# LogicTronixInc/Event-Camera-Clustering-and-Optical-Flow-Estimation

Measured on AMD Instinct MI355X. Metric: Mevents/s (downsample+cluster+corner), higher is better.
Workload: dtype u16xy/i64t (int), fp32 k-means; 1 GPU; e2e hash-downsample(8192-event windows) -> k-means k=16 (10 iters) on reps -> SAE+FAST arc corners (16384-event slices) -> 15x15 NMS; 346x260 sensor; 20004864 events/GPU/step (BASELINE configs C2-C4); events_per_gpu=20004864, events_total=20004864, preset=c4, reps_per_gpu=7697279, width=346, height=260, k=16, kmeans_iters=10, parallelism=time-window shards x1, launch=eager launches, streams=two streams sharing all CUs

## Files before the change

### event-camera-clustering-and-optical-flow-estimation_amd/csrc/corners.hip

```cpp
#include "arc_select.hpp"
#include "corner_decode.hpp"
#include "ecc_internal.hpp"

#include <cstdio>
#include <cstdlib>
#include <map>
#include <mutex>

namespace {

constexpr int kThreads = 256;
constexpr int kBuildUnroll = 8;
constexpr size_t kFlagDynLdsMax = 160 * 1024 - 256;
constexpr int kArcThreads = 512;
constexpr int kGroup = 32;
constexpr int kTile = 14;
constexpr int kTilePix = kTile * kTile;
constexpr int kHalo = 4;
constexpr int kWin = kTile + 2 * kHalo;
constexpr int kWinPix = kWin * kWin;
constexpr int kMaxTiles = 8191;
constexpr int kMaxSlice = 1 << 19;

struct CornerGeom {
// ... 13 lines not shown
    tile = (int)((uint32_t)item - q * (uint32_t)g.n_tiles);
}

struct Sorted {
    uint32_t *key;
    uint32_t *t32;
    int32_t *toff;
};

__constant__ int8_t c3dy[16] = {0, 1, 2, 3, 3, 3, 2, 1, 0, -1, -2, -3, -3, -3, -2, -1};
__constant__ int8_t c3dx[16] = {3, 3, 2, 1, 0, -1, -2, -3, -3, -3, -2, -1, 0, 1, 2, 3};
__constant__ int8_t c4dy[20] = {0, 1, 2, 3, 4, 4, 4, 3, 2, 1, 0, -1, -2, -3, -4, -4, -4, -3, -2, -1};
__constant__ int8_t c4dx[20] = {4, 4, 3, 2, 1, 0, -1, -2, -3, -4, -4, -4, -3, -2, -1, 0, 1, 2, 3, 4};

__device__ __forceinline__ bool is_border(int x, int y, const CornerGeom &g) {
    return x < g.margin || x >= g.W - g.margin || y < g.margin || y >= g.H - g.margin;
}

__device__ __forceinline__ int tile_of(uint32_t v, const CornerGeom &g) {
    const int x = ecc::xy_x(v), y = ecc::xy_y(v);
    const int tl = (int)__umul24((uint32_t)(y / kTile), (uint32_t)g.tiles_x) + x / kTile;
    return (x >= g.W || y >= g.H) ? g.n_tiles : tl;
}

__device__ __forceinline__ uint32_t tile_key(uint32_t v, uint32_t e_local) {
    return (e_local << 8) | (uint32_t)((ecc::xy_y(v) % kTile) * kTile + ecc::xy_x(v) % kTile);
}

__device__ __forceinline__ void tile_origin_xy(const CornerGeom &g, int tile, int &tx, int &ty) {
    ty = (int)magic_quot((uint32_t)tile, g.tx_mul, g.tx_sh);
    tx = tile - ty * g.tiles_x;
// ... 393 lines not shown
    uint32_t r0 = 0u, r1 = 0u, r2 = 0u, r3 = x4;
    uint32_t v = 0u;
    int k = 0;
    for (uint32_t mm = m; mm; mm &= mm - 1u, ++k) {
        v = tab[__ffs(mm) - 1][lp];
        if (k == 0) r0 = v;
        else if (k == 1) r1 = v;
        else if (k == 2) r2 = v;
        else if (cnt == kRecVals) r3 = v;
        else xo[k] = v;
    }
    pv[q] = make_uint4(r0, r1, r2, r3);
    glast[q] = gr.narrow ? gr.Lt + (int64_t)v : t[gr.first + v - 1u];
}

constexpr int kPrefixPix = 64;
constexpr int kPrefixPer = 16;
constexpr int kPrefixRound = kPrefixPer * (kThreads / 64);

__global__ void __launch_bounds__(kThreads)
sae_prefix_kernel(CornerGeom g, int64_t n_groups, const uint32_t *__restrict__ gmask, int64_t *__restrict__ gB,
                  int64_t *__restrict__ sae, int32_t *__restrict__ err_status,
                  int32_t *__restrict__ err_pending, int32_t tag,
                  uint32_t *__restrict__ zero0, int32_t *__restrict__ zero1) {
    if (blockIdx.x == 0 && threadIdx.x == 0) {
        *err_status = *err_pending == tag ? 1 : 0;
        *err_pending = 0;
        if (zero0) *zero0 = 0u;
        if (zero1) *zero1 = 0;
    }
    __shared__ int64_t s_last[kThreads / 64][kPrefixPix];
    __shared__ uint8_t s_has[kThreads / 64][kPrefixPix];
    const int lane = threadIdx.x & 63, wave = threadIdx.x >> 6;
    const int64_t HW = (int64_t)g.H * g.W;
    const int64_t q = (int64_t)blockIdx.x * kPrefixPix + lane;
    const bool in = q < HW;
    int64_t carry = in ? sae[q] : 0;
    for (int64_t r0 = 0; r0 < n_groups; r0 += kPrefixRound) {
        const int64_t g0 = r0 + (int64_t)wave * kPrefixPer;
        uint32_t m[kPrefixPer];
        int64_t lt[kPrefixPer];
#pragma unroll
        for (int u = 0; u < kPrefixPer; ++u) m[u] = (in && g0 + u < n_groups) ? gmask[(g0 + u) * HW + q] : 0u;
#pragma unroll
        for (int u = 0; u < kPrefixPer; ++u) lt[u] = m[u] ? gB[(g0 + u) * HW + q] : 0;
        bool has = false;
        int64_t last = 0;
#pragma unroll
        for (int u = 0; u < kPrefixPer; ++u) {
            if (m[u]) { has = true; last = lt[u]; }
        }
        s_last[wave][lane] = last;
        s_has[wave][lane] = has ? 1 : 0;
        __syncthreads();
        int64_t run = carry;
        for (int w = 0; w < wave; ++w)
            if (s_has[w][lane]) run = s_last[w][lane];
#pragma unroll
        for (int u = 0; u < kPrefixPer; ++u) {
            if (!in || g0 + u >= n_groups) break;
            gB[(g0 + u) * HW + q] = run;
            if (m[u]) run = lt[u];
        }
#pragma unroll
        for (int w = 0; w < kThreads / 64; ++w)
            if (s_has[w][lane]) carry = s_last[w][lane];
        __syncthreads();
    }
    if (in && wave == 0) sae[q] = carry;
}

__global__ void __launch_bounds__(kThreads)
sae_local_last_kernel(CornerGeom g, int64_t n_groups, const uint32_t *__restrict__ gmask,
                      const int64_t *__restrict__ glast, int64_t *__restrict__ out) {
    const int64_t HW = (int64_t)g.H * g.W;
    for (int64_t q = (int64_t)blockIdx.x * kThreads + threadIdx.x; q < HW; q += (int64_t)gridDim.x * kThreads) {
        int64_t run = 0;
        for (int64_t gi = n_groups - 1; gi >= 0; --gi)
            if (gmask[gi * HW + q]) { run = glast[gi * HW + q]; break; }
        out[q] = run;
    }
}


constexpr int kPairWords = kGroup * kTilePix / 32;
constexpr int kSegWords = (kTilePix + 31) / 32;

__device__ __forceinline__ void store_res_slice_major(const uint32_t *bits, int64_t grp, int tile, const CornerGeom &g,
                                                      uint32_t *__restrict__ res, int tid) {
    if (tid >= kGroup * kSegWords) return;
    const int j = tid / kSegWords, w = tid % kSegWords;
    const int b0 = j * kTilePix + 32 * w, w0 = b0 >> 5, sh = b0 & 31;
    uint32_t v = bits[w0] >> sh;
    if (sh && w0 + 1 < kPairWords) v |= bits[w0 + 1] << (32 - sh);
    if (w == kSegWords - 1) v &= (1u << (kTilePix - 32 * (kSegWords - 1))) - 1u;
    res[(grp * kGroup + j) * g.seg_stride + tile * kSegWords + w] = v;
}
constexpr int kWaves = kArcThreads / 64;
constexpr int kQ4Cap = 1024;

struct MaskB {
    uint32_t mask;
    uint32_t bc;
};

struct ArcLds {
    uint32_t T[kGroup][kWinPix];
    MaskB mb[kWinPix];
    uint32_t res[kPairWords];
    uint16_t tasks[kGroup * kTilePix];
    uint16_t q4[kQ4Cap];
    int64_t wave_min[16];
    int32_t exact_only;
    int32_t mixed;
    int32_t q4n;
    int32_t n_exact;
    int32_t wave_own[16];
    int32_t wave_tasks[16];
};

__device__ __forceinline__ uint32_t clamp_rel(int64_t v, int64_t L, int64_t vz, int32_t *exact_flag,
                                              int32_t *mixed_flag) {
    if (v <= L) {
        if (v != vz) *mixed_flag = 1;
        return 0u;
    }
    const int64_t d = v - L;
    if (d > (int64_t)kVMax) { *exact_flag = 1; return kVMax; }
    return (uint32_t)d;
}

__device__ __forceinline__ int64_t readlane_i64(int64_t v, int l) {
    return (int64_t)((uint64_t)__builtin_amdgcn_readlane((uint32_t)((uint64_t)v >> 32), l) << 32 |
                     (uint64_t)__builtin_amdgcn_readlane((uint32_t)v, l));
}
__device__ __forceinline__ void clamp_wave_flags(int64_t bq, int64_t Lt, int64_t &c0, int &cf) {
    const bool clp = bq <= Lt;
    const uint64_t cball = __ballot(clp);
    c0 = 0;
    cf = 0;
    if (cball) {
        c0 = readlane_i64(bq, __ffsll((unsigned long long)cball) - 1);
        cf = 2 | (__ballot(clp && bq != c0) != 0ull ? 1 : 0);
    }
}
template <int W>
__device__ __forceinline__ bool clamp_mixed(const int64_t *wc0, const int32_t *wcf, int lane) {
    const int wf = lane < W ? wcf[lane] : 0;
    const int64_t wv = lane < W ? wc0[lane] : 0;
    const uint64_t has = __ballot(wf & 2);
    bool mixed = __ballot(wf & 1) != 0ull;
    if (has) {
        const int64_t v0 = readlane_i64(wv, __ffsll((unsigned long long)has) - 1);
        mixed = mixed || __ballot((wf & 2) && wv != v0) != 0ull;
    }
    return mixed;
}
__device__ __forceinline__ uint32_t clamp_value(int64_t bq, int64_t Lt, bool narrow, int32_t *exact_flag) {
    if (!narrow || bq == INT64_MAX || bq <= Lt) return 0u;
    const int64_t d = bq - Lt;
    if (d > (int64_t)kVMax) {
        *exact_flag = 1;
        return kVMax;
    }
    return (uint32_t)d;
}

__device__ __forceinline__ uint32_t below_mask(int j) { return (2u << j) - 1u; }

__device__ __forceinline__ uint32_t win_value(const ArcLds &L, int wp, uint32_t below) {
    const MaskB m = L.mb[wp];
    const uint32_t mk = m.mask & below;
    return mk ? L.T[31 - __clz(mk)][wp] : m.bc;
}

struct ExactCtx {
    const int64_t *Bg;
    const int64_t *t;
    int64_t grp_first, Lt;
    int W;
    bool narrow;
};

__device__ __forceinline__ int64_t double_key(int64_t v) {
    const int64_t b = __builtin_bit_cast(int64_t, (double)v);
    return b ^ ((b >> 63) & INT64_MAX);
}

template <int N>
__device__ __forceinline__ void exact_values(const ArcLds *L, int wp0, int64_t q0, uint32_t below,
                                             const int8_t *dy, const int8_t *dx, const ExactCtx &c, int64_t (&v)[N]) {
#pragma unroll
    for (int k = 0; k < N; ++k) {
        if (k > 0 && k % 4 == 0) __builtin_amdgcn_sched_barrier(0);
        const int wp = wp0 + dy[k] * kWin + dx[k];
        const uint32_t mk = L->mb[wp].mask & below;
        const uint32_t tv = mk ? L->T[31 - __clz(mk)][wp] : 0u;
        v[k] = double_key(!mk        ? c.Bg[q0 + (int64_t)dy[k] * c.W + dx[k]]
                          : c.narrow ? c.Lt + (int64_t)tv
                                     : c.t[c.grp_first + tv - 1u]);
    }
}


__device__ __noinline__ bool exact_pair_test(const ArcLds *L, int wp0, int64_t q0, uint32_t below, bool c3_passed,
                                             const int64_t *Bg, const int64_t *t, int64_t grp_first, int64_t Lt, int W,
                                             bool narrow) {
    const ExactCtx c{Bg, t, grp_first, Lt, W, narrow};
    if (!c3_passed) {
        int64_t v3[16];
        exact_values<16>(L, wp0, q0, below, c3dy, c3dx, c, v3);
        if (!arc_streak<16, 3, 6>(v3)) return false;
    }
    int64_t v4[20];
    exact_values<20>(L, wp0, q0, below, c4dy, c4dx, c, v4);
    return arc_streak<20, 4, 8>(v4);
}


__device__ __forceinline__ uint32_t eligible_slices(const CornerGeom &g, int64_t grp) {
    const int gs = (int)grp * kGroup;
    if (g.first_detect <= gs) return 0xffffffffu;
    const int j0 = g.first_detect - gs;
// ... 27 lines not shown
#define DENSE_MARK(k)                                                                \
    do {                                                                             \
        if (tid == 0) {                                                              \
            const unsigned long long now_ = wall_clock64();                          \
            atomicAdd(&g_dense_prof[k], now_ - dense_t_);                            \
            dense_t_ = now_;                                                         \
        }                                                                            \
    } while (0)
#else
#define DENSE_MARK(k) do { } while (0)
#endif

template <int NT>
__device__ __forceinline__ void arc_dense_item(ArcLds &L, int64_t item, const int64_t *__restrict__ t, const CornerGeom &g,
                                               const uint32_t *__restrict__ ovf, const uint4 *__restrict__ pv,
                                               const int64_t *__restrict__ gB, const uint32_t *__restrict__ gmask,
                                               uint32_t *__restrict__ res, const GroupRec *__restrict__ grec) {
    int64_t grp;
    int tile;
    item_decode(g, item, grp, tile);
    if ((int)grp < (g.first_detect >> 5)) return;
    const int tid = threadIdx.x, lane = tid & 63, wave = tid >> 6;
#if ECC_ARC_PROFILE
    const unsigned long long dense_t0_ = wall_clock64();
    unsigned long long dense_t_ = dense_t0_;
#endif
    const int64_t HW = (int64_t)g.H * g.W;
    int tx, ty;
    tile_origin_xy(g, tile, tx, ty);
    const int x0 = tx * kTile, y0 = ty * kTile;
    const GroupRef gr = group_ref_of(grec[grp]);
    const int64_t grp_first = gr.first, Lt = gr.Lt;
    const bool narrow = gr.narrow;
    const int64_t *Bg = gB + grp * HW;

    static_assert(NT >= kWinPix, "one lane per window pixel");
    const int wp = tid;
    const bool win_lane = wp < kWinPix;
    const int ox = wp % kWin - kHalo, oy = wp / kWin - kHalo;
    const int wx = x0 + ox, wy = y0 + oy;
    const bool in = win_lane && wx >= 0 && wy >= 0 && wx < g.W && wy < g.H;
    const int64_t q = grp * HW + (int64_t)wy * g.W + wx;
    int64_t bq = INT64_MAX;
    uint32_t mk = 0u;
    uint4 rec = make_uint4(0u, 0u, 0u, 0u);
    if (in) {
        bq = gB[q];
        mk = gmask[q];
        rec = pv[q];
    }
    for (int w = tid; w < kPairWords; w += NT) L.res[w] = 0u;
    if (tid == 0) {
        L.exact_only = narrow ? 0 : 1;
        L.mixed = 0;
        L.q4n = 0;
        L.n_exact = 0;
    }
    const bool own = win_lane && ox >= 0 && oy >= 0 && ox < kTile && oy < kTile;
    const uint64_t own_pairs = __ballot(own && mk != 0u);
    if (lane == 0) L.wave_own[wave] = own_pairs != 0ull;
    const uint32_t tm0 = (own && !is_border(wx, wy, g)) ? (mk & eligible_slices(g, grp)) : 0u;
    const int tcnt = __popc(tm0);
    const int tincl = ecc::wave_incl_scan(tcnt);
    if (lane == 63) L.wave_tasks[wave] = tincl;
    __syncthreads();
    if (win_lane) {
        L.mb[wp].mask = mk;
        const int p = __popc(mk);
        uint32_t mm = mk;
        for (int k = 0; mm && k < kRecVals - 1; ++k, mm &= mm - 1u)
            L.T[__ffs(mm) - 1][wp] = k == 0 ? rec.x : (k == 1 ? rec.y : rec.z);
        if (mm && p == kRecVals) {
            L.T[__ffs(mm) - 1][wp] = rec.w;
        } else if (mm) {
            overflow_lines(ovf, rec, 0, p, [&](int, uint32_t v) {
                L.T[__ffs(mm) - 1][wp] = v;
                mm &= mm - 1u;
            });
        }
    }
    int toff = tincl - tcnt, n_tasks = 0;
#pragma unroll
    for (int w = 0; w < NT / 64; ++w) {
        const int c = L.wave_tasks[w];
        toff += w < wave ? c : 0;
        n_tasks += c;
    }
    for (uint32_t tm = tm0; tm; tm &= tm - 1u) L.tasks[toff++] = (uint16_t)((__ffs(tm) - 1) << 9 | wp);
    const int64_t bmin = ecc::wave_min_i64(bq);
    if (lane == 0) L.wave_min[wave] = bmin;
    __syncthreads();
    DENSE_MARK(0);
    {
        int any = 0;
#pragma unroll
        for (int w = 0; w < NT / 64; ++w) any |= L.wave_own[w];
        if (!any) return;
    }
    DENSE_MARK(1);

    if (win_lane) {
        int64_t vz = INT64_MAX;
#pragma unroll
        for (int w = 0; w < NT / 64; ++w) vz = L.wave_min[w] < vz ? L.wave_min[w] : vz;
        L.mb[wp].bc = (!narrow || bq == INT64_MAX) ? 0u : clamp_rel(bq, Lt, vz, &L.exact_only, &L.mixed);
    }
    __syncthreads();
    DENSE_MARK(2);

    const bool fast = !L.exact_only;
    const bool ties_exact = !L.mixed;
    constexpr uint16_t kOpen3 = 0x4000, kOpen4 = 0x8000;
    if (fast) {
        for (int ti = tid; ti < n_tasks; ti += NT) {
            const int pi = L.tasks[ti];
            const int wp0 = pi & 511;
            const uint32_t below = below_mask(pi >> 9);
            uint32_t k3[16];
#pragma unroll
            for (int k = 0; k < 16; ++k) k3[k] = (win_value(L, wp0 + c3dy[k] * kWin + c3dx[k], below) << 5) | k;
            const int r3 = arc_keys<16, 5, 3, 6>(k3, ties_exact);
            if (r3 > 0) {
                const int qi = atomicAdd(&L.q4n, 1);
                if (qi < kQ4Cap) L.q4[qi] = (uint16_t)ti;
                else { L.tasks[ti] = (uint16_t)(pi | kOpen4); L.n_exact = 1; }
// ... 4 lines not shown
        }
    }
    __syncthreads();
    DENSE_MARK(3);
    const int n4 = min(L.q4n, kQ4Cap);
    for (int qi = tid; qi < n4; qi += NT) {
        const int ti = L.q4[qi];
        const int pi = L.tasks[ti];
        const int j = pi >> 9, wp0 = pi & 511;
        const uint32_t below = below_mask(j);
        uint32_t k4[20];
#pragma unroll
        for (int k = 0; k < 20; ++k) k4[k] = (win_value(L, wp0 + c4dy[k] * kWin + c4dx[k], below) << 5) | k;
        const int r4 = arc_keys<20, 5, 4, 8>(k4, ties_exact);
        if (r4 > 0) {
            const int rb = j * kTilePix + (wp0 / kWin - kHalo) * kTile + (wp0 % kWin - kHalo);
            atomicOr(&L.res[rb >> 5], 1u << (rb & 31));
        } else if (r4 < 0) {
            L.tasks[ti] = (uint16_t)(pi | kOpen4);
            L.n_exact = 1;
        }
    }
    __syncthreads();
    DENSE_MARK(4);
    if (!fast || L.n_exact) {
        for (int ti = tid; ti < n_tasks; ti += NT) {
            const int e = L.tasks[ti], pi = e & 0x3fff;
            if (fast && !(e & (kOpen3 | kOpen4))) continue;
            const int j = pi >> 9, wp0 = pi & 511;
            const int ly = wp0 / kWin - kHalo, lx = wp0 % kWin - kHalo;
            const int64_t q0 = (int64_t)(y0 + ly) * g.W + (x0 + lx);
            const uint32_t below = below_mask(j);
            if (exact_pair_test(&L, wp0, q0, below, (e & kOpen4) != 0, Bg, t, grp_first, Lt, g.W, narrow)) {
                const int rb = j * kTilePix + ly * kTile + lx;
                atomicOr(&L.res[rb >> 5], 1u << (rb & 31));
            }
        }
        __syncthreads();
    }
#if ECC_ARC_PROFILE
    if (tid == 0) {
        atomicMax(&g_dense_prof[5], wall_clock64() - dense_t0_);
        atomicAdd(&g_dense_prof[6], (unsigned long long)n_tasks);
        atomicAdd(&g_dense_prof[7], 1ull);
    }
#endif
    store_res_slice_major(L.res, grp, tile, g, res, tid);
}

// ... 3 lines not shown
constexpr int kValCap = ECC_ARC_VALCAP;

struct PixInfo {
    uint32_t mask;
    uint32_t off;
};

struct SparseLds {
    uint32_t vals[kValCap + kWinPix];
    PixInfo pix[kWinPix];
    uint32_t res[kPairWords];
    uint16_t tasks[kValCap];
    uint16_t q4[kQ4Cap];
    int64_t wave_c0[kWaves];
    int32_t wave_cf[kWaves];
    int32_t wave_tot[kWaves];
    int32_t exact_only, mixed, q4n, redo;
};

static_assert(sizeof(PixInfo) == 8, "one 8-B LDS read per pixel");
__device__ __forceinline__ uint32_t sparse_value(const SparseLds &L, int wp, uint32_t below) {
    const uint2 p = reinterpret_cast<const uint2 *>(L.pix)[wp];
    return L.vals[p.y + __popc(p.x & below)];
}

#ifndef ECC_ARC_SKIP_OVF
#define ECC_ARC_SKIP_OVF 0
#endif
#ifndef ECC_ARC_WAVES
#define ECC_ARC_WAVES 8
#endif

// ... 1 lines not shown
constexpr int kProfItems = 1 << 15;
__device__ unsigned long long g_arc_items[kProfItems][8];
#define ARC_MARK(k)                                                                  \
    do {                                                                             \
        if (tid == 0) {                                                              \
            const unsigned long long now_ = wall_clock64();                          \
            arc_ph_[k] = now_ - arc_t_;                                              \
            arc_t_ = now_;                                                           \
        }                                                                            \
    } while (0)
#else
#define ARC_MARK(k) do { } while (0)
#endif

struct ArcPre {
    int64_t bq;
    uint32_t mk;
    uint4 rec;
};

__device__ __forceinline__ void arc_prefetch(ArcPre &p, int64_t item, const CornerGeom &g, const uint4 *__restrict__ pv,
                                             const int64_t *__restrict__ gB, const uint32_t *__restrict__ gmask) {
    const int tid = threadIdx.x;
    p.bq = INT64_MAX;
    p.mk = 0u;
    p.rec = make_uint4(0u, 0u, 0u, 0u);
    const int64_t HW = (int64_t)g.H * g.W;
    int64_t grp;
    int tile, tx, ty;
    item_decode(g, item, grp, tile);
    tile_origin_xy(g, tile, tx, ty);
    const int wx = tx * kTile - kHalo + tid % kWin, wy = ty * kTile - kHalo + tid / kWin;
    if (tid < kWinPix && wx >= 0 && wy >= 0 && wx < g.W && wy < g.H) {
        const int64_t q = grp * HW + (int64_t)wy * g.W + wx;
        p.bq = gB[q];
        p.mk = gmask[q];
        p.rec = pv[q];
    }
}

__device__ __forceinline__ void arc_item(SparseLds &L, int64_t item, const ArcPre &pre,
                                         const GroupRec *__restrict__ grec, const CornerGeom &g,
                                         const uint32_t *__restrict__ ovf, uint32_t *__restrict__ res,
                                         int64_t *__restrict__ over, uint32_t *__restrict__ n_over) {
    int64_t grp;
    int tile;
    item_decode(g, item, grp, tile);
    if ((int)grp < (g.first_detect >> 5)) return;
    static_assert(kGroup == 32, "first_detect >> 5");
    const int tid = threadIdx.x, lane = tid & 63, wave = tid >> 6;
    const int wave_s = __builtin_amdgcn_readfirstlane(wave);
#if ECC_ARC_PROFILE
    unsigned long long arc_t_ = wall_clock64(), arc_ph_[8] = {0, 0, 0, 0, 0, 0, 0, 0};
#endif
    int tx, ty;
    tile_origin_xy(g, tile, tx, ty);
    const int x0 = tx * kTile, y0 = ty * kTile;
    const GroupRec rec = grec[grp];
    const int64_t Lt = rec.Lt;
    const bool narrow = (rec.bits & kRecNarrow) != 0u;
    const int wp = tid;
    const bool win_lane = wp < kWinPix;
    const int64_t bq = pre.bq;
    const uint32_t mk_w = pre.mk;
    const int ox = wp % kWin - kHalo, oy = wp / kWin - kHalo;
    const bool own = win_lane && ox >= 0 && oy >= 0 && ox < kTile && oy < kTile;
    for (int w = tid; w < kPairWords; w += kArcThreads) L.res[w] = 0u;
    if (tid == 0) {
        L.exact_only = narrow ? 0 : 1;
        L.q4n = 0;
        L.redo = 0;
    }
    const uint32_t tm = (own && !is_border(x0 + ox, y0 + oy, g)) ? (mk_w & eligible_slices(g, grp)) : 0u;
    const int cnt = win_lane ? __popc(mk_w) + 1 : 0;
    const int tcnt = __popc(tm);
    constexpr int kTaskShift = 14, kOwnShift = 27;
    constexpr int kCntMask = (1 << kTaskShift) - 1, kTaskMask = (1 << (kOwnShift - kTaskShift)) - 1;
    const int both = ecc::wave_incl_scan(tcnt << kTaskShift | cnt);
    const int incl = both & kCntMask, tincl = both >> kTaskShift;
    const uint64_t own_pairs = __ballot(own && mk_w != 0u);
    int64_t c0;
    int cf;
    clamp_wave_flags(bq, Lt, c0, cf);
    const int p = cnt - 1;
#ifndef ECC_ARC_XPF
#define ECC_ARC_XPF 1
#endif
    constexpr int kXpf = ECC_ARC_XPF > 0 ? ECC_ARC_XPF : 1;
    uint4 xs[kXpf];
#pragma unroll
    for (int u = 0; u < kXpf; ++u) xs[u] = make_uint4(0u, 0u, 0u, 0u);
    if (ECC_ARC_XPF && __ballot(p > kRecVals)) {
        const bool o = p > kRecVals;
        const uint4 *x4 = reinterpret_cast<const uint4 *>(ovf) + (o ? pre.rec.w : 0u);
        const int nl = o ? (p - (kRecVals - 1) + 3) >> 2 : 1;
#pragma unroll
        for (int u = 0; u < kXpf; ++u) xs[u] = x4[min(u, nl - 1)];
    }
    if (lane == 63) L.wave_tot[wave] = both | (own_pairs != 0ull ? 1 << kOwnShift : 0);
    if (lane == 0) {
        L.wave_c0[wave] = c0;
        L.wave_cf[wave] = cf;
    }
    __syncthreads();
    ARC_MARK(0);
    int sum = 0, before = 0;
#pragma unroll
    for (int w = 0; w < kWaves; ++w) {
        const int wb = L.wave_tot[w];
        sum += wb;
        before += w < wave_s ? wb : 0;
    }
    const int total = sum & kCntMask, any_own = sum >> kOwnShift;
    int n_tasks = (sum >> kTaskShift) & kTaskMask;
    const int off = incl - cnt + (before & kCntMask);
    int toff = tincl - tcnt + ((before >> kTaskShift) & kTaskMask);
    if (wave == 0) {
        const bool mixed = clamp_mixed<kWaves>(L.wave_c0, L.wave_cf, lane);
        if (lane == 0) L.mixed = mixed;
    }
    if (!any_own || total > kValCap + kWinPix) {
        if (any_own && tid == 0) over[atomicAdd(n_over, 1u)] = item;
        return;
    }
    if (win_lane) {
        const uint32_t bcv = clamp_value(bq, Lt, narrow, &L.exact_only);
        reinterpret_cast<uint2 *>(L.pix)[wp] = make_uint2(mk_w, (uint32_t)off);
        uint32_t *dst = L.vals + off;
        dst[0] = bcv;
        if (p > 0) dst[1] = pre.rec.x;
        if (p > 1) dst[2] = pre.rec.y;
        if (p > 2) dst[3] = pre.rec.z;
        if (p == kRecVals) {
            dst[4] = pre.rec.w;
        } else if (!ECC_ARC_XPF && p > kRecVals) {
            overflow_lines(ovf, pre.rec, 0, p, [&](int k, uint32_t v) { dst[1 + k] = v; });
        } else if (p > kRecVals) {
#pragma unroll
            for (int u = 0; u < kXpf; ++u) {
                const int k = (kRecVals - 1) + 4 * u;
                if (k < p) dst[1 + k] = xs[u].x;
                if (k + 1 < p) dst[2 + k] = xs[u].y;
                if (k + 2 < p) dst[3 + k] = xs[u].z;
                if (k + 3 < p) dst[4 + k] = xs[u].w;
            }
            if (!ECC_ARC_SKIP_OVF && p > kRecVals + 4 * ECC_ARC_XPF - 1)
                overflow_lines(ovf, pre.rec, ECC_ARC_XPF, p, [&](int k, uint32_t v) { dst[1 + k] = v; });
        }
        for (uint32_t m = tm; m; m &= m - 1u) L.tasks[toff++] = (uint16_t)((__ffs(m) - 1) << 9 | wp);
    }
    __syncthreads();
    ARC_MARK(1);
    if (L.exact_only) {
        if (tid == 0) over[atomicAdd(n_over, 1u)] = item;
        return;
    }
#ifndef ECC_ARC_SKIP
#define ECC_ARC_SKIP 0
#endif
    if (ECC_ARC_SKIP >= 2) n_tasks = 0;
    const bool ties_exact = !L.mixed;
    for (int ti = tid; ti < n_tasks; ti += kArcThreads) {
        const int pi = L.tasks[ti];
        const int wp0 = pi & 511;
        const uint32_t below = below_mask(pi >> 9);
        uint32_t k3[16];
#pragma unroll
        for (int k = 0; k < 16; ++k) k3[k] = (sparse_value(L, wp0 + c3dy[k] * kWin + c3dx[k], below) << 5) | k;
        const int r3 = arc_keys<16, 5, 3, 6>(k3, ties_exact);
        if (r3 > 0) {
            const int qi = atomicAdd(&L.q4n, 1);
// ... 13 lines not shown
#if ECC_ARC_PROFILE
    if (tid == 0) {
        arc_ph_[5] = (unsigned long long)n_tasks;
        arc_ph_[6] = (unsigned long long)n4;
    }
#endif
    for (int qi = tid; qi < n4; qi += kArcThreads) {
        const int pt = L.q4[qi];
        const int j = pt >> 9, wp0 = pt & 511;
        const uint32_t below = below_mask(j);
        uint32_t k4[20];
#pragma unroll
        for (int k = 0; k < 20; ++k) k4[k] = (sparse_value(L, wp0 + c4dy[k] * kWin + c4dx[k], below) << 5) | k;
        const int r4 = arc_keys<20, 5, 4, 8>(k4, ties_exact);
        if (r4 > 0) {
            const int pi = j * kTilePix + (wp0 / kWin - kHalo) * kTile + (wp0 % kWin - kHalo);
            atomicOr(&L.res[pi >> 5], 1u << (pi & 31));
        } else if (r4 < 0) {
            L.redo = 1;
        }
    }
    __syncthreads();
    ARC_MARK(4);
#if ECC_ARC_PROFILE
    if (tid == 0 && item < kProfItems) {
        arc_ph_[7] = 1ull;
        for (int k = 0; k < 8; ++k) g_arc_items[item][k] = arc_ph_[k];
    }
#endif
    if (L.redo) {
        if (tid == 0) over[atomicAdd(n_over, 1u)] = item;
        return;
    }
    store_res_slice_major(L.res, grp, tile, g, res, tid);
}

__global__ void __launch_bounds__(kArcThreads, ECC_ARC_WAVES)
arc_kernel(const GroupRec *__restrict__ grec, CornerGeom g, int64_t n_items, const uint32_t *__restrict__ ovf,
           const uint4 *__restrict__ pv, const int64_t *__restrict__ gB, const uint32_t *__restrict__ gmask,
           uint32_t *__restrict__ res, int64_t *__restrict__ over, uint32_t *__restrict__ n_over) {
    __shared__ SparseLds L;
    const int per = (int)(gridDim.x / 8);
    const int64_t item = (int)(blockIdx.x % 8) * per + (int)(blockIdx.x / 8);
    if (item >= n_items) return;
    ArcPre pre;
    arc_prefetch(pre, item, g, pv, gB, gmask);
    arc_item(L, item, pre, grec, g, ovf, res, over, n_over);
}


#ifndef ECC_DENSE_THREADS
#define ECC_DENSE_THREADS 512
#endif
constexpr int kDenseThreads = ECC_DENSE_THREADS;
__global__ void __launch_bounds__(kDenseThreads, 4)
arc_dense_kernel(const int64_t *__restrict__ t, CornerGeom g, const int64_t *__restrict__ over,
                 const uint32_t *__restrict__ n_over, const uint32_t *__restrict__ ovf, const uint4 *__restrict__ pv,
                 const int64_t *__restrict__ gB, const uint32_t *__restrict__ gmask, uint32_t *__restrict__ res,
                 const GroupRec *__restrict__ grec) {
    __shared__ ArcLds L;
    const uint32_t n = *n_over;
    for (uint32_t li = blockIdx.x; li < n; li += gridDim.x) {
        arc_dense_item<kDenseThreads>(L, over[li], t, g, ovf, pv, gB, gmask, res, grec);
        __syncthreads();
    }
}

#ifndef ECC_FLAG_THREADS
#define ECC_FLAG_THREADS 256
#endif
constexpr int kFlagThreads = ECC_FLAG_THREADS;
#ifndef ECC_FLAG_QUADS
#define ECC_FLAG_QUADS 8
#endif
constexpr int kFlagQuads = ECC_FLAG_QUADS;
constexpr int kFlagBatch = kFlagQuads * kFlagThreads;
constexpr int kFlagCandMax = 16384;

// ... 168 lines not shown
        T *r = base ? reinterpret_cast<T *>(base + used) : nullptr;
        used += ecc::align_up(count * sizeof(T), 256);
        return r;
    }
};

struct GroupImages {
    uint32_t *mask;
    int64_t *B;
    uint32_t *res;
    uint4 *pv;
    uint32_t *ovf;
    int64_t *over;
    uint32_t *n_over;
    GroupRec *grec;
};

Sorted carve_sorted(Carve &cv, const CornerGeom &g, int64_t n_items, int64_t n_groups, int32_t **first_border,
                    GroupImages *gi) {
    Sorted so{};
    so.key = cv.take<uint32_t>((size_t)g.n);
    so.t32 = cv.take<uint32_t>((size_t)g.n);
    so.toff = cv.take<int32_t>((size_t)g.n_slices * (g.n_tiles + 2));
    *first_border = cv.take<int32_t>((size_t)g.n_slices);
    const size_t img = (size_t)n_groups * g.W * g.H;
    gi->mask = cv.take<uint32_t>(img);
    gi->B = cv.take<int64_t>(img);
    gi->res = cv.take<uint32_t>((size_t)n_groups * kGroup * g.seg_stride);
    gi->pv = cv.take<uint4>(img);
    gi->ovf = cv.take<uint32_t>((size_t)g.n + 4 * (size_t)n_items + 8);
    gi->over = cv.take<int64_t>((size_t)n_items);
    gi->n_over = cv.take<uint32_t>(64);
    gi->grec = cv.take<GroupRec>((size_t)n_groups);
    return so;
}

int corner_state_reserve(ecc_ctx *ctx, CornerState *st, size_t evt_need) {
    if (evt_need > st->evt_bytes) {
        if (st->evt) {
            ECC_CHECK_HIP(ctx, hipDeviceSynchronize(), "sync(corner batch)");
            (void)hipFree(st->evt);
            st->evt = nullptr;
            st->evt_bytes = 0;
            st->n_over = nullptr;
        }
        const size_t want = ecc::align_up(evt_need + evt_need / 8, 1 << 20);
        hipError_t e = hipMalloc(&st->evt, want);
        if (e != hipSuccess) {
// ... 134 lines not shown
    if (!(phases & 2)) {
        st->status_src = 1;
        ECC_CHECK_LAUNCH(ctx, "fast_detect_prepare");
        return ECC_OK;
    }
    st->status_src = 2;
    st->n_over = gi.n_over;
    st->n_items = n_items;
    st->n_slices = g.n_slices;
    st->n_groups = n_groups;
    {
        ECC_TIMED(ctx, s, "sae_prefix_kernel");
        const int64_t HW = (int64_t)g.W * g.H;
        const unsigned blocks = (unsigned)((HW + kPrefixPix - 1) / kPrefixPix);
        hipLaunchKernelGGL(sae_prefix_kernel, dim3(blocks), dim3(kThreads), 0, s, g, n_groups,
                           (const uint32_t *)gi.mask, gi.B, sae, &ctx->dev->fast_verdict, &ctx->dev->sort_pending,
                           st->prep_tag, (phases & 1) ? nullptr : gi.n_over, (phases & 1) ? nullptr : zero_nms_err);
    }
    {
        ECC_TIMED(ctx, s, "arc_kernel");
        {
            const unsigned grid = (unsigned)(8 * ((n_items + 7) / 8));
            hipLaunchKernelGGL(arc_kernel, dim3(grid), dim3(kArcThreads), 0, s, (const GroupRec *)gi.grec, g, n_items,
                               (const uint32_t *)gi.ovf, (const uint4 *)gi.pv, (const int64_t *)gi.B, (const uint32_t *)gi.mask, gi.res, gi.over, gi.n_over);
        }
    }
    {
        ECC_TIMED(ctx, s, "arc_dense_kernel");
        hipLaunchKernelGGL(arc_dense_kernel, dim3(kDenseThreads == 512 ? 512 : ctx->n_cu), dim3(kDenseThreads), 0, s, t, g, (const int64_t *)gi.over,
                           (const uint32_t *)gi.n_over, (const uint32_t *)gi.ovf, (const uint4 *)gi.pv,
                           (const int64_t *)gi.B, (const uint32_t *)gi.mask, gi.res, (const GroupRec *)gi.grec);
    }
    {
        ECC_TIMED(ctx, s, "flags_kernel");
        constexpr size_t kLdsMax = kFlagDynLdsMax;
        const size_t lds = (size_t)g.n_tiles * kSegWords * sizeof(uint32_t);
        if (lds <= kLdsMax) {
            static bool lds_set[2] = {false, false};
            const void *fn = cand ? reinterpret_cast<const void *>(&flags_event_kernel<true, true>)
                                  : reinterpret_cast<const void *>(&flags_event_kernel<true, false>);
            if (lds > 65536 && !lds_set[cand ? 1 : 0]) {
                ECC_CHECK_HIP(ctx, hipFuncSetAttribute(fn, hipFuncAttributeMaxDynamicSharedMemorySize, (int)kLdsMax),
                              "flags LDS");
                lds_set[cand ? 1 : 0] = true;
            }
            if (cand)
// ... 169 lines not shown
```

Before: 43460 Mevents/s.

## Stage packed mask/clamped-value/border words in SAE prefix for arc kernels

The SAE prefix kernel now writes a packed uint2 per pixel and group. It holds the slice mask plus a 32-bit word with the clamped relative timestamp and low, exact and border flags. The 64-bit B value is stored only when the word cannot encode it. The arc and dense kernels then read one 8-byte word instead of separate 64-bit B and 32-bit mask loads, skip border recomputation, and find exact_only earlier. Result bits are laid out per slice on word-aligned strides, which simplifies the stores. The cost is an extra staging buffer, extra work in the prefix kernel, and a smaller per-round group count.

```diff
diff --git a/event-camera-clustering-and-optical-flow-estimation_amd/csrc/arc_stage_word.hpp b/event-camera-clustering-and-optical-flow-estimation_amd/csrc/arc_stage_word.hpp
--- /dev/null
+++ b/event-camera-clustering-and-optical-flow-estimation_amd/csrc/arc_stage_word.hpp
@@ -0,0 +1,30 @@
+#pragma once
+#include <cstdint>
+
+#if defined(__HIPCC__) || defined(__CUDACC__)
+#define ECC_STAGE_HD __host__ __device__ inline __attribute__((always_inline))
+#else
+#define ECC_STAGE_HD inline
+#endif
+
+constexpr int kStageValueBits = 27;
+constexpr uint32_t kStageValueMax = (1u << kStageValueBits) - 1u;
+constexpr uint32_t kStageLow = 1u << 27;
+constexpr uint32_t kStageExact = 1u << 28;
+constexpr uint32_t kStageBorder = 1u << 29;
+constexpr uint32_t kStageNeedsB = kStageLow | kStageExact;
+
+ECC_STAGE_HD constexpr bool stage_is_border(int x, int y, int W, int H, int margin) {
+    return x < margin || x >= W - margin || y < margin || y >= H - margin;
+}
+
+ECC_STAGE_HD constexpr uint32_t stage_value_bits(int64_t b, int64_t lt, bool narrow) {
+    if (!narrow) return kStageExact;
+    if (b <= lt) return kStageLow;
+    const uint64_t d = (uint64_t)b - (uint64_t)lt;
+    return d > (uint64_t)kStageValueMax ? (kStageValueMax | kStageExact) : (uint32_t)d;
+}
+
+ECC_STAGE_HD constexpr uint32_t stage_word(int64_t b, int64_t lt, bool narrow, bool border) {
+    return stage_value_bits(b, lt, narrow) | (border ? kStageBorder : 0u);
+}
diff --git a/event-camera-clustering-and-optical-flow-estimation_amd/csrc/corners.hip b/event-camera-clustering-and-optical-flow-estimation_amd/csrc/corners.hip
--- a/event-camera-clustering-and-optical-flow-estimation_amd/csrc/corners.hip
+++ b/event-camera-clustering-and-optical-flow-estimation_amd/csrc/corners.hip
@@ -1,4 +1,5 @@
 #include "arc_select.hpp"
+#include "arc_stage_word.hpp"
 #include "corner_decode.hpp"
 #include "ecc_internal.hpp"
 
@@ -51,7 +52,7 @@
 __constant__ int8_t c4dx[20] = {4, 4, 3, 2, 1, 0, -1, -2, -3, -4, -4, -4, -3, -2, -1, 0, 1, 2, 3, 4};
 
 __device__ __forceinline__ bool is_border(int x, int y, const CornerGeom &g) {
-    return x < g.margin || x >= g.W - g.margin || y < g.margin || y >= g.H - g.margin;
+    return stage_is_border(x, y, g.W, g.H, g.margin);
 }
 
 __device__ __forceinline__ int tile_of(uint32_t v, const CornerGeom &g) {
@@ -475,12 +476,19 @@
     glast[q] = gr.narrow ? gr.Lt + (int64_t)v : t[gr.first + v - 1u];
 }
 
+__device__ __forceinline__ int64_t readlane_i64(int64_t v, int l) {
+    const uint32_t hi = (uint32_t)__builtin_amdgcn_readlane((int)(uint32_t)((uint64_t)v >> 32), l);
+    const uint32_t lo = (uint32_t)__builtin_amdgcn_readlane((int)(uint32_t)v, l);
+    return (int64_t)((uint64_t)hi << 32 | (uint64_t)lo);
+}
+
 constexpr int kPrefixPix = 64;
-constexpr int kPrefixPer = 16;
+constexpr int kPrefixPer = 12;
 constexpr int kPrefixRound = kPrefixPer * (kThreads / 64);
 
 __global__ void __launch_bounds__(kThreads)
 sae_prefix_kernel(CornerGeom g, int64_t n_groups, const uint32_t *__restrict__ gmask, int64_t *__restrict__ gB,
+                  uint2 *__restrict__ gw, const GroupRec *__restrict__ grec,
                   int64_t *__restrict__ sae, int32_t *__restrict__ err_status,
                   int32_t *__restrict__ err_pending, int32_t tag,
                   uint32_t *__restrict__ zero0, int32_t *__restrict__ zero1) {
@@ -492,10 +500,12 @@
     }
     __shared__ int64_t s_last[kThreads / 64][kPrefixPix];
     __shared__ uint8_t s_has[kThreads / 64][kPrefixPix];
-    const int lane = threadIdx.x & 63, wave = threadIdx.x >> 6;
+    const int lane = threadIdx.x & 63, wave = __builtin_amdgcn_readfirstlane(threadIdx.x >> 6);
     const int64_t HW = (int64_t)g.H * g.W;
     const int64_t q = (int64_t)blockIdx.x * kPrefixPix + lane;
     const bool in = q < HW;
+    const int py = (int)((uint32_t)q / (uint32_t)g.W), px = (int)((uint32_t)q - (uint32_t)py * (uint32_t)g.W);
+    const uint32_t border_bit = is_border(px, py, g) ? kStageBorder : 0u;
     int64_t carry = in ? sae[q] : 0;
     for (int64_t r0 = 0; r0 < n_groups; r0 += kPrefixRound) {
         const int64_t g0 = r0 + (int64_t)wave * kPrefixPer;
@@ -505,6 +515,10 @@
         for (int u = 0; u < kPrefixPer; ++u) m[u] = (in && g0 + u < n_groups) ? gmask[(g0 + u) * HW + q] : 0u;
 #pragma unroll
         for (int u = 0; u < kPrefixPer; ++u) lt[u] = m[u] ? gB[(g0 + u) * HW + q] : 0;
+        static_assert(kPrefixPer <= 32, "one lane per group of the round, their verdicts in a 32-bit mask");
+        const GroupRec &my_rec = grec[min(g0 + (lane % kPrefixPer), n_groups - 1)];
+        const int64_t my_lt = my_rec.Lt;
+        const uint32_t narrow_groups = (uint32_t)__ballot((my_rec.bits & kRecNarrow) != 0u);
         bool has = false;
         int64_t last = 0;
 #pragma unroll
@@ -520,7 +534,9 @@
 #pragma unroll
         for (int u = 0; u < kPrefixPer; ++u) {
             if (!in || g0 + u >= n_groups) break;
-            gB[(g0 + u) * HW + q] = run;
+            const uint32_t vb = stage_value_bits(run, readlane_i64(my_lt, u), ((narrow_groups >> u) & 1u) != 0u);
+            gw[(g0 + u) * HW + q] = make_uint2(m[u], vb | border_bit);
+            if (vb & kStageNeedsB) gB[(g0 + u) * HW + q] = run;
             if (m[u]) run = lt[u];
         }
 #pragma unroll
@@ -544,18 +560,15 @@
 }
 
 
-constexpr int kPairWords = kGroup * kTilePix / 32;
 constexpr int kSegWords = (kTilePix + 31) / 32;
+constexpr int kSliceBits = kSegWords * 32;
+constexpr int kPairWords = kGroup * kSegWords;
 
 __device__ __forceinline__ void store_res_slice_major(const uint32_t *bits, int64_t grp, int tile, const CornerGeom &g,
                                                       uint32_t *__restrict__ res, int tid) {
     if (tid >= kGroup * kSegWords) return;
     const int j = tid / kSegWords, w = tid % kSegWords;
-    const int b0 = j * kTilePix + 32 * w, w0 = b0 >> 5, sh = b0 & 31;
-    uint32_t v = bits[w0] >> sh;
-    if (sh && w0 + 1 < kPairWords) v |= bits[w0 + 1] << (32 - sh);
-    if (w == kSegWords - 1) v &= (1u << (kTilePix - 32 * (kSegWords - 1))) - 1u;
-    res[(grp * kGroup + j) * g.seg_stride + tile * kSegWords + w] = v;
+    res[(grp * kGroup + j) * g.seg_stride + tile * kSegWords + w] = bits[tid];
 }
 constexpr int kWaves = kArcThreads / 64;
 constexpr int kQ4Cap = 1024;
@@ -571,8 +584,9 @@
     uint32_t res[kPairWords];
     uint16_t tasks[kGroup * kTilePix];
     uint16_t q4[kQ4Cap];
-    int64_t wave_min[16];
-    int32_t exact_only;
+    int64_t wave_c0[16];
+    int32_t wave_cf[16];
+    int32_t wave_ex[16];
     int32_t mixed;
     int32_t q4n;
     int32_t n_exact;
@@ -580,21 +594,8 @@
     int32_t wave_tasks[16];
 };
 
-__device__ __forceinline__ uint32_t clamp_rel(int64_t v, int64_t L, int64_t vz, int32_t *exact_flag,
-                                              int32_t *mixed_flag) {
-    if (v <= L) {
-        if (v != vz) *mixed_flag = 1;
-        return 0u;
-    }
-    const int64_t d = v - L;
-    if (d > (int64_t)kVMax) { *exact_flag = 1; return kVMax; }
-    return (uint32_t)d;
-}
-
-__device__ __forceinline__ int64_t readlane_i64(int64_t v, int l) {
-    return (int64_t)((uint64_t)__builtin_amdgcn_readlane((uint32_t)((uint64_t)v >> 32), l) << 32 |
-                     (uint64_t)__builtin_amdgcn_readlane((uint32_t)v, l));
-}
+static_assert(kStageValueMax == kVMax, "the staging word's key is the clamped value of the tests");
+
 __device__ __forceinline__ void clamp_wave_flags(int64_t bq, int64_t Lt, int64_t &c0, int &cf) {
     const bool clp = bq <= Lt;
     const uint64_t cball = __ballot(clp);
@@ -617,14 +618,19 @@
     }
     return mixed;
 }
-__device__ __forceinline__ uint32_t clamp_value(int64_t bq, int64_t Lt, bool narrow, int32_t *exact_flag) {
-    if (!narrow || bq == INT64_MAX || bq <= Lt) return 0u;
-    const int64_t d = bq - Lt;
-    if (d > (int64_t)kVMax) {
-        *exact_flag = 1;
-        return kVMax;
-    }
-    return (uint32_t)d;
+__device__ __forceinline__ int64_t stage_b_of(uint32_t bw, int64_t Lt, const int64_t *__restrict__ bq_at) {
+    return (bw & kStageNeedsB) ? *bq_at : Lt + (int64_t)(bw & kStageValueMax);
+}
+
+template <class Addr>
+__device__ __forceinline__ void stage_wave_flags(uint32_t bw, Addr bq_at, int64_t Lt, int64_t &c0, int &cf) {
+    c0 = 0;
+    cf = 0;
+    if (__ballot(bw & kStageLow)) {
+        int64_t bq = INT64_MAX;
+        if (bw & kStageLow) bq = *bq_at();
+        clamp_wave_flags(bq, Lt, c0, cf);
+    }
 }
 
 __device__ __forceinline__ uint32_t below_mask(int j) { return (2u << j) - 1u; }
@@ -637,6 +643,7 @@
 
 struct ExactCtx {
     const int64_t *Bg;
+    const uint2 *Wg;
     const int64_t *t;
     int64_t grp_first, Lt;
     int W;
@@ -657,7 +664,8 @@
         const int wp = wp0 + dy[k] * kWin + dx[k];
         const uint32_t mk = L->mb[wp].mask & below;
         const uint32_t tv = mk ? L->T[31 - __clz(mk)][wp] : 0u;
-        v[k] = double_key(!mk        ? c.Bg[q0 + (int64_t)dy[k] * c.W + dx[k]]
+        const int64_t qn = q0 + (int64_t)dy[k] * c.W + dx[k];
+        v[k] = double_key(!mk        ? stage_b_of(c.Wg[qn].y, c.Lt, c.Bg + qn)
                           : c.narrow ? c.Lt + (int64_t)tv
                                      : c.t[c.grp_first + tv - 1u]);
     }
@@ -665,9 +673,9 @@
 
 
 __device__ __noinline__ bool exact_pair_test(const ArcLds *L, int wp0, int64_t q0, uint32_t below, bool c3_passed,
-                                             const int64_t *Bg, const int64_t *t, int64_t grp_first, int64_t Lt, int W,
-                                             bool narrow) {
-    const ExactCtx c{Bg, t, grp_first, Lt, W, narrow};
+                                             const int64_t *Bg, const uint2 *Wg, const int64_t *t, int64_t grp_first,
+                                             int64_t Lt, int W, bool narrow) {
+    const ExactCtx c{Bg, Wg, t, grp_first, Lt, W, narrow};
     if (!c3_passed) {
         int64_t v3[16];
         exact_values<16>(L, wp0, q0, below, c3dy, c3dx, c, v3);
@@ -725,7 +733,7 @@
 template <int NT>
 __device__ __forceinline__ void arc_dense_item(ArcLds &L, int64_t item, const int64_t *__restrict__ t, const CornerGeom &g,
                                                const uint32_t *__restrict__ ovf, const uint4 *__restrict__ pv,
-                                               const int64_t *__restrict__ gB, const uint32_t *__restrict__ gmask,
+                                               const int64_t *__restrict__ gB, const uint2 *__restrict__ gw,
                                                uint32_t *__restrict__ res, const GroupRec *__restrict__ grec) {
     int64_t grp;
     int tile;
@@ -752,31 +760,28 @@
     const int wx = x0 + ox, wy = y0 + oy;
     const bool in = win_lane && wx >= 0 && wy >= 0 && wx < g.W && wy < g.H;
     const int64_t q = grp * HW + (int64_t)wy * g.W + wx;
-    int64_t bq = INT64_MAX;
-    uint32_t mk = 0u;
+    uint2 sw = make_uint2(0u, 0u);
     uint4 rec = make_uint4(0u, 0u, 0u, 0u);
     if (in) {
-        bq = gB[q];
-        mk = gmask[q];
+        sw = gw[q];
         rec = pv[q];
     }
+    const uint32_t mk = sw.x, bw = sw.y;
     for (int w = tid; w < kPairWords; w += NT) L.res[w] = 0u;
     if (tid == 0) {
-        L.exact_only = narrow ? 0 : 1;
-        L.mixed = 0;
         L.q4n = 0;
         L.n_exact = 0;
     }
     const bool own = win_lane && ox >= 0 && oy >= 0 && ox < kTile && oy < kTile;
     const uint64_t own_pairs = __ballot(own && mk != 0u);
     if (lane == 0) L.wave_own[wave] = own_pairs != 0ull;
-    const uint32_t tm0 = (own && !is_border(wx, wy, g)) ? (mk & eligible_slices(g, grp)) : 0u;
+    const uint32_t tm0 = (own && !(bw & kStageBorder)) ? (mk & eligible_slices(g, grp)) : 0u;
     const int tcnt = __popc(tm0);
     const int tincl = ecc::wave_incl_scan(tcnt);
     if (lane == 63) L.wave_tasks[wave] = tincl;
     __syncthreads();
     if (win_lane) {
-        L.mb[wp].mask = mk;
+        reinterpret_cast<uint2 *>(L.mb)[wp] = make_uint2(mk, bw & kVMax);
         const int p = __popc(mk);
         uint32_t mm = mk;
         for (int k = 0; mm && k < kRecVals - 1; ++k, mm &= mm - 1u)
@@ -798,8 +803,17 @@
         n_tasks += c;
     }
     for (uint32_t tm = tm0; tm; tm &= tm - 1u) L.tasks[toff++] = (uint16_t)((__ffs(tm) - 1) << 9 | wp);
-    const int64_t bmin = ecc::wave_min_i64(bq);
-    if (lane == 0) L.wave_min[wave] = bmin;
+    {
+        int64_t c0;
+        int cf;
+        stage_wave_flags(bw, [&] { return gB + q; }, Lt, c0, cf);
+        const uint64_t exb = __ballot(bw & kStageExact);
+        if (lane == 0) {
+            L.wave_c0[wave] = c0;
+            L.wave_cf[wave] = cf;
+            L.wave_ex[wave] = exb != 0ull;
+        }
+    }
     __syncthreads();
     DENSE_MARK(0);
     {
@@ -810,16 +824,17 @@
     }
     DENSE_MARK(1);
 
-    if (win_lane) {
-        int64_t vz = INT64_MAX;
-#pragma unroll
-        for (int w = 0; w < NT / 64; ++w) vz = L.wave_min[w] < vz ? L.wave_min[w] : vz;
-        L.mb[wp].bc = (!narrow || bq == INT64_MAX) ? 0u : clamp_rel(bq, Lt, vz, &L.exact_only, &L.mixed);
+    int exact_only = 0;
+#pragma unroll
+    for (int w = 0; w < NT / 64; ++w) exact_only |= L.wave_ex[w];
+    if (wave == 0) {
+        const bool mixed = clamp_mixed<NT / 64>(L.wave_c0, L.wave_cf, lane);
+        if (lane == 0) L.mixed = mixed;
     }
     __syncthreads();
     DENSE_MARK(2);
 
-    const bool fast = !L.exact_only;
+    const bool fast = !exact_only;
     const bool ties_exact = !L.mixed;
     constexpr uint16_t kOpen3 = 0x4000, kOpen4 = 0x8000;
     if (fast) {
@@ -854,7 +869,7 @@
         for (int k = 0; k < 20; ++k) k4[k] = (win_value(L, wp0 + c4dy[k] * kWin + c4dx[k], below) << 5) | k;
         const int r4 = arc_keys<20, 5, 4, 8>(k4, ties_exact);
         if (r4 > 0) {
-            const int rb = j * kTilePix + (wp0 / kWin - kHalo) * kTile + (wp0 % kWin - kHalo);
+            const int rb = j * kSliceBits + (wp0 / kWin - kHalo) * kTile + (wp0 % kWin - kHalo);
             atomicOr(&L.res[rb >> 5], 1u << (rb & 31));
         } else if (r4 < 0) {
             L.tasks[ti] = (uint16_t)(pi | kOpen4);
@@ -871,8 +886,8 @@
             const int ly = wp0 / kWin - kHalo, lx = wp0 % kWin - kHalo;
             const int64_t q0 = (int64_t)(y0 + ly) * g.W + (x0 + lx);
             const uint32_t below = below_mask(j);
-            if (exact_pair_test(&L, wp0, q0, below, (e & kOpen4) != 0, Bg, t, grp_first, Lt, g.W, narrow)) {
-                const int rb = j * kTilePix + ly * kTile + lx;
+            if (exact_pair_test(&L, wp0, q0, below, (e & kOpen4) != 0, Bg, gw + grp * HW, t, grp_first, Lt, g.W, narrow)) {
+                const int rb = j * kSliceBits + ly * kTile + lx;
                 atomicOr(&L.res[rb >> 5], 1u << (rb & 31));
             }
         }
@@ -906,8 +921,8 @@
     uint16_t q4[kQ4Cap];
     int64_t wave_c0[kWaves];
     int32_t wave_cf[kWaves];
-    int32_t wave_tot[kWaves];
-    int32_t exact_only, mixed, q4n, redo;
+    uint32_t wave_tot[kWaves];
+    int32_t mixed, q4n, redo;
 };
 
 static_assert(sizeof(PixInfo) == 8, "one 8-B LDS read per pixel");
@@ -939,16 +954,14 @@
 #endif
 
 struct ArcPre {
-    int64_t bq;
-    uint32_t mk;
+    uint2 sw;
     uint4 rec;
 };
 
 __device__ __forceinline__ void arc_prefetch(ArcPre &p, int64_t item, const CornerGeom &g, const uint4 *__restrict__ pv,
-                                             const int64_t *__restrict__ gB, const uint32_t *__restrict__ gmask) {
+                                             const uint2 *__restrict__ gw) {
     const int tid = threadIdx.x;
-    p.bq = INT64_MAX;
-    p.mk = 0u;
+    p.sw = make_uint2(0u, 0u);
     p.rec = make_uint4(0u, 0u, 0u, 0u);
     const int64_t HW = (int64_t)g.H * g.W;
     int64_t grp;
@@ -958,16 +971,16 @@
     const int wx = tx * kTile - kHalo + tid % kWin, wy = ty * kTile - kHalo + tid / kWin;
     if (tid < kWinPix && wx >= 0 && wy >= 0 && wx < g.W && wy < g.H) {
         const int64_t q = grp * HW + (int64_t)wy * g.W + wx;
-        p.bq = gB[q];
-        p.mk = gmask[q];
+        p.sw = gw[q];
         p.rec = pv[q];
     }
 }
 
 __device__ __forceinline__ void arc_item(SparseLds &L, int64_t item, const ArcPre &pre,
                                          const GroupRec *__restrict__ grec, const CornerGeom &g,
-                                         const uint32_t *__restrict__ ovf, uint32_t *__restrict__ res,
-                                         int64_t *__restrict__ over, uint32_t *__restrict__ n_over) {
+                                         const uint32_t *__restrict__ ovf, const int64_t *__restrict__ gB,
+                                         uint32_t *__restrict__ res, int64_t *__restrict__ over,
+                                         uint32_t *__restrict__ n_over) {
     int64_t grp;
     int tile;
     item_decode(g, item, grp, tile);
@@ -983,30 +996,29 @@
     const int x0 = tx * kTile, y0 = ty * kTile;
     const GroupRec rec = grec[grp];
     const int64_t Lt = rec.Lt;
-    const bool narrow = (rec.bits & kRecNarrow) != 0u;
     const int wp = tid;
     const bool win_lane = wp < kWinPix;
-    const int64_t bq = pre.bq;
-    const uint32_t mk_w = pre.mk;
+    const uint32_t mk_w = pre.sw.x, bw = pre.sw.y;
     const int ox = wp % kWin - kHalo, oy = wp / kWin - kHalo;
     const bool own = win_lane && ox >= 0 && oy >= 0 && ox < kTile && oy < kTile;
     for (int w = tid; w < kPairWords; w += kArcThreads) L.res[w] = 0u;
     if (tid == 0) {
-        L.exact_only = narrow ? 0 : 1;
         L.q4n = 0;
         L.redo = 0;
     }
-    const uint32_t tm = (own && !is_border(x0 + ox, y0 + oy, g)) ? (mk_w & eligible_slices(g, grp)) : 0u;
+    const uint32_t tm = (own && !(bw & kStageBorder)) ? (mk_w & eligible_slices(g, grp)) : 0u;
     const int cnt = win_lane ? __popc(mk_w) + 1 : 0;
     const int tcnt = __popc(tm);
-    constexpr int kTaskShift = 14, kOwnShift = 27;
+    constexpr int kTaskShift = 14, kOwnShift = 27, kExactShift = 31;
     constexpr int kCntMask = (1 << kTaskShift) - 1, kTaskMask = (1 << (kOwnShift - kTaskShift)) - 1;
+    constexpr int kOwnMask = (1 << (kExactShift - kOwnShift)) - 1;
     const int both = ecc::wave_incl_scan(tcnt << kTaskShift | cnt);
     const int incl = both & kCntMask, tincl = both >> kTaskShift;
     const uint64_t own_pairs = __ballot(own && mk_w != 0u);
+    const uint64_t exact_words = __ballot(bw & kStageExact);
     int64_t c0;
     int cf;
-    clamp_wave_flags(bq, Lt, c0, cf);
+    stage_wave_flags(bw, [&] { return gB + (grp * ((int64_t)g.H * g.W) + (int64_t)(y0 + oy) * g.W + (x0 + ox)); }, Lt, c0, cf);
     const int p = cnt - 1;
 #ifndef ECC_ARC_XPF
 #define ECC_ARC_XPF 1
@@ -1022,37 +1034,39 @@
 #pragma unroll
         for (int u = 0; u < kXpf; ++u) xs[u] = x4[min(u, nl - 1)];
     }
-    if (lane == 63) L.wave_tot[wave] = both | (own_pairs != 0ull ? 1 << kOwnShift : 0);
+    if (lane == 63)
+        L.wave_tot[wave] = (uint32_t)both | (own_pairs != 0ull ? 1u << kOwnShift : 0u) | (exact_words != 0ull ? 1u << kExactShift : 0u);
     if (lane == 0) {
         L.wave_c0[wave] = c0;
         L.wave_cf[wave] = cf;
     }
     __syncthreads();
     ARC_MARK(0);
-    int sum = 0, before = 0;
+    uint32_t sum = 0u, before = 0u, any = 0u;
 #pragma unroll
     for (int w = 0; w < kWaves; ++w) {
-        const int wb = L.wave_tot[w];
+        const uint32_t wb = L.wave_tot[w];
         sum += wb;
-        before += w < wave_s ? wb : 0;
-    }
-    const int total = sum & kCntMask, any_own = sum >> kOwnShift;
-    int n_tasks = (sum >> kTaskShift) & kTaskMask;
-    const int off = incl - cnt + (before & kCntMask);
-    int toff = tincl - tcnt + ((before >> kTaskShift) & kTaskMask);
+        any |= wb;
+        before += w < wave_s ? wb : 0u;
+    }
+    const int total = (int)(sum & kCntMask), any_own = (int)((sum >> kOwnShift) & kOwnMask);
+    const bool exact_only = (any >> kExactShift) != 0u;
+    int n_tasks = (int)((sum >> kTaskShift) & kTaskMask);
+    const int off = incl - cnt + (int)(before & kCntMask);
+    int toff = tincl - tcnt + (int)((before >> kTaskShift) & kTaskMask);
     if (wave == 0) {
         const bool mixed = clamp_mixed<kWaves>(L.wave_c0, L.wave_cf, lane);
         if (lane == 0) L.mixed = mixed;
     }
-    if (!any_own || total > kValCap + kWinPix) {
+    if (!any_own || exact_only || total > kValCap + kWinPix) {
         if (any_own && tid == 0) over[atomicAdd(n_over, 1u)] = item;
         return;
     }
     if (win_lane) {
-        const uint32_t bcv = clamp_value(bq, Lt, narrow, &L.exact_only);
         reinterpret_cast<uint2 *>(L.pix)[wp] = make_uint2(mk_w, (uint32_t)off);
         uint32_t *dst = L.vals + off;
-        dst[0] = bcv;
+        dst[0] = bw & kVMax;
         if (p > 0) dst[1] = pre.rec.x;
         if (p > 1) dst[2] = pre.rec.y;
         if (p > 2) dst[3] = pre.rec.z;
@@ -1076,10 +1090,6 @@
     }
     __syncthreads();
     ARC_MARK(1);
-    if (L.exact_only) {
-        if (tid == 0) over[atomicAdd(n_over, 1u)] = item;
-        return;
-    }
 #ifndef ECC_ARC_SKIP
 #define ECC_ARC_SKIP 0
 #endif
@@ -1123,7 +1133,7 @@
         for (int k = 0; k < 20; ++k) k4[k] = (sparse_value(L, wp0 + c4dy[k] * kWin + c4dx[k], below) << 5) | k;
         const int r4 = arc_keys<20, 5, 4, 8>(k4, ties_exact);
         if (r4 > 0) {
-            const int pi = j * kTilePix + (wp0 / kWin - kHalo) * kTile + (wp0 % kWin - kHalo);
+            const int pi = j * kSliceBits + (wp0 / kWin - kHalo) * kTile + (wp0 % kWin - kHalo);
             atomicOr(&L.res[pi >> 5], 1u << (pi & 31));
         } else if (r4 < 0) {
             L.redo = 1;
@@ -1146,15 +1156,15 @@
 
 __global__ void __launch_bounds__(kArcThreads, ECC_ARC_WAVES)
 arc_kernel(const GroupRec *__restrict__ grec, CornerGeom g, int64_t n_items, const uint32_t *__restrict__ ovf,
-           const uint4 *__restrict__ pv, const int64_t *__restrict__ gB, const uint32_t *__restrict__ gmask,
+           const uint4 *__restrict__ pv, const int64_t *__restrict__ gB, const uint2 *__restrict__ gw,
            uint32_t *__restrict__ res, int64_t *__restrict__ over, uint32_t *__restrict__ n_over) {
     __shared__ SparseLds L;
     const int per = (int)(gridDim.x / 8);
     const int64_t item = (int)(blockIdx.x % 8) * per + (int)(blockIdx.x / 8);
     if (item >= n_items) return;
     ArcPre pre;
-    arc_prefetch(pre, item, g, pv, gB, gmask);
-    arc_item(L, item, pre, grec, g, ovf, res, over, n_over);
+    arc_prefetch(pre, item, g, pv, gw);
+    arc_item(L, item, pre, grec, g, ovf, gB, res, over, n_over);
 }
 
 
@@ -1165,12 +1175,12 @@
 __global__ void __launch_bounds__(kDenseThreads, 4)
 arc_dense_kernel(const int64_t *__restrict__ t, CornerGeom g, const int64_t *__restrict__ over,
                  const uint32_t *__restrict__ n_over, const uint32_t *__restrict__ ovf, const uint4 *__restrict__ pv,
-                 const int64_t *__restrict__ gB, const uint32_t *__restrict__ gmask, uint32_t *__restrict__ res,
+                 const int64_t *__restrict__ gB, const uint2 *__restrict__ gw, uint32_t *__restrict__ res,
                  const GroupRec *__restrict__ grec) {
     __shared__ ArcLds L;
     const uint32_t n = *n_over;
     for (uint32_t li = blockIdx.x; li < n; li += gridDim.x) {
-        arc_dense_item<kDenseThreads>(L, over[li], t, g, ovf, pv, gB, gmask, res, grec);
+        arc_dense_item<kDenseThreads>(L, over[li], t, g, ovf, pv, gB, gw, res, grec);
         __syncthreads();
     }
 }
@@ -1369,6 +1379,7 @@
     int64_t *over;
     uint32_t *n_over;
     GroupRec *grec;
+    uint2 *gw;
 };
 
 Sorted carve_sorted(Carve &cv, const CornerGeom &g, int64_t n_items, int64_t n_groups, int32_t **first_border,
@@ -1387,6 +1398,7 @@
     gi->over = cv.take<int64_t>((size_t)n_items);
     gi->n_over = cv.take<uint32_t>(64);
     gi->grec = cv.take<GroupRec>((size_t)n_groups);
+    gi->gw = cv.take<uint2>(img);
     return so;
 }
 
@@ -1551,7 +1563,8 @@
         const int64_t HW = (int64_t)g.W * g.H;
         const unsigned blocks = (unsigned)((HW + kPrefixPix - 1) / kPrefixPix);
         hipLaunchKernelGGL(sae_prefix_kernel, dim3(blocks), dim3(kThreads), 0, s, g, n_groups,
-                           (const uint32_t *)gi.mask, gi.B, sae, &ctx->dev->fast_verdict, &ctx->dev->sort_pending,
+                           (const uint32_t *)gi.mask, gi.B, gi.gw, (const GroupRec *)gi.grec, sae, &ctx->dev->fast_verdict,
+                           &ctx->dev->sort_pending,
                            st->prep_tag, (phases & 1) ? nullptr : gi.n_over, (phases & 1) ? nullptr : zero_nms_err);
     }
     {
@@ -1559,14 +1572,15 @@
         {
             const unsigned grid = (unsigned)(8 * ((n_items + 7) / 8));
             hipLaunchKernelGGL(arc_kernel, dim3(grid), dim3(kArcThreads), 0, s, (const GroupRec *)gi.grec, g, n_items,
-                               (const uint32_t *)gi.ovf, (const uint4 *)gi.pv, (const int64_t *)gi.B, (const uint32_t *)gi.mask, gi.res, gi.over, gi.n_over);
+                               (const uint32_t *)gi.ovf, (const uint4 *)gi.pv, (const int64_t *)gi.B, (const uint2 *)gi.gw,
+                               gi.res, gi.over, gi.n_over);
         }
     }
     {
         ECC_TIMED(ctx, s, "arc_dense_kernel");
         hipLaunchKernelGGL(arc_dense_kernel, dim3(kDenseThreads == 512 ? 512 : ctx->n_cu), dim3(kDenseThreads), 0, s, t, g, (const int64_t *)gi.over,
                            (const uint32_t *)gi.n_over, (const uint32_t *)gi.ovf, (const uint4 *)gi.pv,
-                           (const int64_t *)gi.B, (const uint32_t *)gi.mask, gi.res, (const GroupRec *)gi.grec);
+                           (const int64_t *)gi.B, (const uint2 *)gi.gw, gi.res, (const GroupRec *)gi.grec);
     }
     {
         ECC_TIMED(ctx, s, "flags_kernel");
```

After: 43460 Mevents/s. About the same (-0.0%).
